# ThorsteinnJonsson/SLAM_framework

Hardware: AMD Instinct MI355X
Metric: stereo frames/sec ORB extract+match @1241x376, 2000 kp/frame (higher is better)
Workload: dtype u8; 1 GPU; configs[1]: synthetic 1241x376 stereo stream, 2000 kp/frame, extract L+R + stereo match + frame-to-frame match; batch=256, streams=1, batches_in_flight=2, nfeatures=2000, nlevels=8, parallelism=frame-sharded x1

## Files before the change

slam_framework_amd/csrc/match_kernels.hip:

```cpp
#include <hip/hip_runtime.h>
#include <stdint.h>

#include "device_math.h"
#include "timing.h"
#include "match_kernels.h"
#include "undistort.h"

namespace slamgpu {

#ifndef STEREO_LANES
#define STEREO_LANES 16
#endif

constexpr int TH_HIGH = 100, TH_LOW = 50, HISTO_LENGTH = 30;
constexpr uint64_t kNoKey = ~0ull;

__device__ __forceinline__ int hamming32(const uint8_t* a, const uint8_t* b) {
  const uint64_t* pa = reinterpret_cast<const uint64_t*>(a);
  const uint64_t* pb = reinterpret_cast<const uint64_t*>(b);
  return __popcll(pa[0] ^ pb[0]) + __popcll(pa[1] ^ pb[1]) + __popcll(pa[2] ^ pb[2]) +
         __popcll(pa[3] ^ pb[3]);
}

__device__ __forceinline__ const uint8_t* level_img(const ImageBatch& b, const OrbGeom* g,
                                                    int img, int level, int* pitch) {
  if (level == 0) {
    *pitch = b.in_pitch;
    return batch_image(b, img);
  }
  *pitch = g->lv[level].pitch;
  return b.pyr + (int64_t)img * g->pyr_bytes + g->lv[level].offset;
}

template <int CAP, int NT = 256>
__device__ int scan256(int* arr, int n, int* wsum) {
  constexpr int per = (CAP + NT - 1) / NT;
  const int lane = threadIdx.x & 63, wid = wave_id();
  const int base = threadIdx.x * per;
  int loc[per];
  int s = 0;
#pragma unroll
  for (int i = 0; i < per; i++) {
    loc[i] = (base + i < n) ? arr[base + i] : 0;
    s += loc[i];
  }
  int x = s;
#pragma unroll
  for (int off = 1; off < 64; off <<= 1) {
    const int y = __shfl_up(x, off, 64);
    if (lane >= off) x += y;
  }
  if (lane == 63) wsum[wid] = x;
  __syncthreads();
  int pre = 0, tot = 0;
#pragma unroll
  for (int w = 0; w < NT / 64; w++) {
    pre += (w < wid) ? wsum[w] : 0;
    tot += wsum[w];
  }
  pre += x - s;
#pragma unroll
  for (int i = 0; i < per; i++) {
    if (base + i < n) arr[base + i] = pre;
    pre += loc[i];
  }
  __syncthreads();
  return tot;
}

__device__ __forceinline__ uint32_t wave_or(uint32_t v) {
#pragma unroll
  for (int off = 32; off >= 1; off >>= 1) v |= __shfl_xor(v, off, 64);
  return v;
}

constexpr int kMaxRows = 2048;

template <int NT>
__device__ __forceinline__ void stereo_rows_body(int f, const OrbGeom* __restrict__ g,
                                                 const FrameKps& ext, int nrows,
                                                 const StereoWorkspace& ws,
                                                 uint32_t* __restrict__ err) {
  __shared__ int cnt[kMaxRows + 1];
  __shared__ int wsum[NT / 64];
  const int tid = threadIdx.x;
  const int ir = 2 * f + 1;
  const KeyPoint* kr = ext.kps + ir * ext.stride;
  const int nr = ext.n[ir * ext.n_stride];
  int* rs = ws.row_start + (int64_t)f * (nrows + 1);
  uint2* items = ws.row_items + (int64_t)f * ws.row_cap;
  for (int i = tid; i <= nrows; i += NT) cnt[i] = 0;
  __syncthreads();
  constexpr int kChunk = 2048 / NT;
  uint2 kit[kChunk];
  auto row_span = [&](int base, int (&lo)[kChunk], int (&hi)[kChunk]) {
    float ky[kChunk];
    int ko[kChunk];
#pragma unroll
    for (int u = 0; u < kChunk; u++) {
      const int i = base + NT * u + tid;
      ky[u] = 0.0f;
      ko[u] = -1;
      if (i < nr) {
        ky[u] = kr[i].y;
        ko[u] = kr[i].octave;
        kit[u] = make_uint2((uint32_t)i | (uint32_t)ko[u] << 16, __float_as_uint(kr[i].x));
      }
    }
#pragma unroll
    for (int u = 0; u < kChunk; u++) {
      lo[u] = 0;
      hi[u] = -1;
      if (ko[u] >= 0) {
        const float r = 2.0f * g->lv[ko[u]].scale;
        lo[u] = max((int)floorf(ky[u] - r), 0);
        hi[u] = min((int)ceilf(ky[u] + r), nrows - 1);
      }
    }
  };
  for (int base = 0; base < nr; base += NT * kChunk) {
    int lo[kChunk], hi[kChunk];
    row_span(base, lo, hi);
#pragma unroll
    for (int u = 0; u < kChunk; u++)
      for (int yi = lo[u]; yi <= hi[u]; ++yi) atomicAdd(&cnt[yi], 1);
  }
  __syncthreads();
  const int total = scan256<kMaxRows + 1, NT>(cnt, nrows, wsum);
  for (int i = tid; i < nrows; i += NT) rs[i] = cnt[i];
  if (tid == 0) {
    rs[nrows] = total;
    if (total > ws.row_cap) atomicOr(err, kErrRowOverflow);
  }
  __syncthreads();
  for (int base = 0; base < nr; base += NT * kChunk) {
    int lo[kChunk], hi[kChunk];
    row_span(base, lo, hi);
#pragma unroll
    for (int u = 0; u < kChunk; u++)
      for (int yi = lo[u]; yi <= hi[u]; ++yi) {
        const int pos = atomicAdd(&cnt[yi], 1);
        if (pos < ws.row_cap) items[pos] = kit[u];
      }
  }
}

template <int NT>
__global__ __launch_bounds__(NT) void stereo_rows_kernel(const OrbGeom* __restrict__ g,
                                                         FrameKps ext, int nrows,
                                                         StereoWorkspace ws,
                                                         uint32_t* __restrict__ err) {
  stereo_rows_body<NT>(blockIdx.x, g, ext, nrows, ws, err);
}

template <int G>
__device__ __forceinline__ uint32_t group_min(uint32_t v) {
#pragma unroll
  for (int off = G / 2; off >= 1; off >>= 1) {
    const uint32_t o = __shfl_xor(v, off, 64);
    v = o < v ? o : v;
  }
  return v;
}

template <int G>
__global__ __launch_bounds__(256) void stereo_match_kernel(ImageBatch b,
                                                           const OrbGeom* __restrict__ g,
                                                           FrameKps ext, Camera cam, int nrows,
                                                           StereoWorkspace ws, StereoOut out) {
  constexpr int NPW = 64 / G;
  constexpr int kRounds = (121 + G - 1) / G;
  int f, bx;
  xcd_image_block(&f, &bx);
  const int lane = threadIdx.x & 63, grp = lane / G, hl = lane % G;
  const int iL = (bx * 4 + wave_id()) * NPW + grp;
  const int il = 2 * f, ir = 2 * f + 1;
  const int nl = ext.n[il * ext.n_stride];
  const int64_t o = (int64_t)f * g->kp_cap + iL;
  bool ok = iL < nl;
  if (ok && hl == 0) {
    out.u_right[o] = -1.0f;
    out.depth[o] = -1.0f;
    ws.sad[o] = -1;
  }
  KeyPoint kpL{};
  if (ok) kpL = ext.kps[il * ext.stride + iL];
  const int levelL = kpL.octave;
  const float vL = kpL.y, uL = kpL.x;
  const int row = (int)vL;
  ok = ok && row >= 0 && row < nrows;
  const int* rs = ws.row_start + (int64_t)f * (nrows + 1);
  const uint2* items = ws.row_items + (int64_t)f * ws.row_cap;
  int c0 = 0, c1 = 0;
  if (ok) {
    c0 = rs[row];
    c1 = min(rs[row + 1], ws.row_cap);
  }
  ok = ok && c0 < c1;
  const float baseline = cam.bf / cam.fx;
  const float minZ = baseline, minD = 0, maxD = cam.bf / minZ;
  const float minU = uL - maxD, maxU = uL - minD;
  ok = ok && !(maxU < 0);
  const uint8_t* dL = ext.desc + (il * ext.stride + (ok ? iL : 0)) * 32;
  const uint8_t* dRb = ext.desc + ir * ext.stride * 32;
  uint32_t best = ((uint32_t)TH_HIGH << 16) | 0xffffu;
  float bestU = 0.0f;
  if (ok) {
    constexpr int kCandU = 2;
    const uint4* dLq = reinterpret_cast<const uint4*>(dL);
    const uint4 l0 = dLq[0], l1 = dLq[1];
    for (int cb = c0 + hl; cb < c1; cb += G * kCandU) {
      int iR[kCandU];
      float uR[kCandU];
      bool pass[kCandU];
#pragma unroll
      for (int u = 0; u < kCandU; u++) {
        const int c = cb + G * u;
        const uint2 it = c < c1 ? items[c] : make_uint2(0xffffffffu, 0u);
        iR[u] = (int)(it.x & 0xffffu);
        const int oct = (int)(it.x >> 16);
        uR[u] = __uint_as_float(it.y);
        pass[u] = c < c1 && oct >= levelL - 1 && oct <= levelL + 1 && uR[u] >= minU &&
                  uR[u] <= maxU;
      }
      uint4 r0[kCandU], r1[kCandU];
#pragma unroll
      for (int u = 0; u < kCandU; u++)
        if (pass[u]) {
          const uint4* dr = reinterpret_cast<const uint4*>(dRb + iR[u] * 32);
          r0[u] = dr[0];
          r1[u] = dr[1];
        }
#pragma unroll
      for (int u = 0; u < kCandU; u++)
        if (pass[u]) {
          const int dist = __popc(l0.x ^ r0[u].x) + __popc(l0.y ^ r0[u].y) + __popc(l0.z ^ r0[u].z) +
                           __popc(l0.w ^ r0[u].w) + __popc(l1.x ^ r1[u].x) + __popc(l1.y ^ r1[u].y) +
                           __popc(l1.z ^ r1[u].z) + __popc(l1.w ^ r1[u].w);
          const uint32_t key = ((uint32_t)dist << 16) | (uint32_t)iR[u];
          if (dist < TH_HIGH && key < best) {
            best = key;
            bestU = uR[u];
          }
        }
    }
  }
  const uint32_t mine = best;
  best = group_min<G>(best);
  const uint64_t gmask = (G == 64 ? ~0ull : ((1ull << G) - 1ull)) << (G * grp);
  const uint64_t hit = __ballot(mine == best) & gmask;
  const float uRbest = __shfl(bestU, hit ? __builtin_ctzll(hit) : lane, 64);
  const int bestDist = (int)(best >> 16);
  const int thOrbDist = (TH_HIGH + TH_LOW) / 2;
  ok = ok && bestDist < thOrbDist;
  const float uR0 = ok ? uRbest : 0.f;
  const float scaleFactor = g->lv[levelL].inv_scale;
  const float scaleduL = roundf(kpL.x * scaleFactor);
  const float scaledvL = roundf(kpL.y * scaleFactor);
  const float scaleduR0 = roundf(uR0 * scaleFactor);
  const int w = 5, L = 5;
  const LevelGeom& LG = g->lv[levelL];
  const float iniu = scaleduR0 + L - w;
  const float endu = scaleduR0 + L + w + 1;
  ok = ok && !(iniu < 0 || endu >= (float)LG.w);
  const int yc = (int)scaledvL, xcl = (int)scaleduL, xcr = (int)scaleduR0;
  ok = ok && !(yc - w < 0 || yc + w >= LG.h || xcl - w < 0 || xcl + w >= LG.w || xcr - L - w < 0);
  __shared__ int s_part[4][NPW][128];
  __shared__ uint32_t s_win[4][NPW][11][11];
  int* part = s_part[wave_id()][grp];
  uint32_t(*win)[11] = s_win[wave_id()][grp];
  int pl = 0, pr = 0;
  const uint8_t* IL = nullptr;
  const uint8_t* IR = nullptr;
  if (ok) {
    IL = level_img(b, g, il, levelL, &pl);
    IR = level_img(b, g, ir, levelL, &pr);
  }
  const int al = (xcl - w) & ~3, ar = (xcr - L - w) & ~3;
  const bool dw = ((((uintptr_t)IL | (uintptr_t)IR) | (uintptr_t)(pl | pr)) & 3) == 0;
  const int lastw = (LG.w - 1) >> 2;
  if (ok) {
#pragma unroll
    for (int rnd = 0; rnd < kRounds; rnd++) {
      const int p = hl + G * rnd;
      if (p < 121) {
        const int r = p / 11, d = p - 11 * r;
        const bool left = d < 4;
        const uint8_t* img = left ? IL : IR;
        const int pitch = left ? pl : pr;
        const int x0 = left ? al + 4 * d : ar + 4 * (d - 4);
        const uint8_t* rowp = img + (int64_t)(yc - w + r) * pitch;
        uint32_t v;
        if (dw) {
          v = reinterpret_cast<const uint32_t*>(rowp)[min(x0 >> 2, lastw)];
        } else {
          v = 0;
          for (int j = 0; j < 4; j++)
            v |= (uint32_t)rowp[min(x0 + j, LG.w - 1)] << (8 * j);
        }
        win[r][d] = v;
      }
    }
  }
  __builtin_amdgcn_fence(__ATOMIC_SEQ_CST, "wavefront");
  __builtin_amdgcn_wave_barrier();
  const uint8_t* wb = reinterpret_cast<const uint8_t*>(&win[0][0]);
  if (ok) {
    const uint32_t* ww = &win[0][0];
    const int oL = xcl - w - al, oR0 = xcr - L - w - ar;
    const int cl = wb[44 * w + (xcl - al)];
    constexpr uint32_t kBias = 0x02020202u;
#pragma unroll
    for (int rnd = 0; rnd < kRounds; rnd++) {
      const int p = hl + G * rnd;
      if (p < 121) {
        const int k = p / 11, yr = p - 11 * k;
        const int cr = wb[44 * w + 16 + (xcr + k - L - ar)];
        const uint32_t* rowL = ww + 11 * yr;
        const int oR = oR0 + k;
        const uint32_t* rowR = rowL + 4 + (oR >> 2);
        const uint32_t l0 = rowL[0], l1 = rowL[1], l2 = rowL[2], l3 = rowL[3];
        const uint32_t r0 = rowR[0], r1 = rowR[1], r2 = rowR[2], r3 = rowR[3];
        const uint32_t a[3] = {__builtin_amdgcn_alignbyte(l1, l0, oL),
                               __builtin_amdgcn_alignbyte(l2, l1, oL),
                               __builtin_amdgcn_alignbyte(l3, l2, oL)};
        const uint32_t bsh = (uint32_t)(oR & 3);
        const uint32_t bb[3] = {__builtin_amdgcn_alignbyte(r1, r0, bsh),
                                __builtin_amdgcn_alignbyte(r2, r1, bsh),
                                __builtin_amdgcn_alignbyte(r3, r2, bsh)};
        typedef unsigned short u16x2_t __attribute__((ext_vector_type(2)));
        const unsigned short d = (unsigned short)(cl - cr);
        const u16x2_t dd = {d, d}, dlast = {d, 0};
        uint32_t acc = 0;
#pragma unroll
        for (int j = 0; j < 6; j++) {
          const uint32_t sel = j == 5 ? 0x04040402u : (j & 1) ? 0x04030402u : 0x05010400u;
          const uint32_t A = __builtin_amdgcn_perm(kBias, a[j >> 1], sel);
          const u16x2_t B = __builtin_bit_cast(u16x2_t, __builtin_amdgcn_perm(kBias, bb[j >> 1], sel)) +
                            (j == 5 ? dlast : dd);
          acc = __builtin_amdgcn_sad_u16(A, __builtin_bit_cast(uint32_t, B), acc);
        }
        part[p] = (int)acc;
      }
    }
  }
  __builtin_amdgcn_fence(__ATOMIC_SEQ_CST, "wavefront");
  __builtin_amdgcn_wave_barrier();
  int sad = 0x7fffffff;
  if (ok && hl < 2 * L + 1) {
    int acc = 0;
#pragma unroll
    for (int yy = 0; yy < 2 * w + 1; yy++) acc += part[11 * hl + yy];
    sad = acc;
  }
  float vDists[11];
#pragma unroll
  for (int k = 0; k < 11; k++) vDists[k] = (float)__shfl(sad, G * grp + k, 64);
  if (!ok || hl != 0) return;
  int bestSad = 0x7fffffff, bestincR = 0;
#pragma unroll
  for (int k = 0; k < 11; k++) {
    if (vDists[k] < (float)bestSad) {
      bestSad = (int)vDists[k];
      bestincR = k - L;
    }
  }
  if (bestincR == -L || bestincR == L) return;
  const float dist1 = vDists[L + bestincR - 1];
  const float dist2 = vDists[L + bestincR];
  const float dist3 = vDists[L + bestincR + 1];
  const float deltaR = (dist1 - dist3) / (2.0f * (dist1 + dist3 - 2.0f * dist2));
  if (deltaR < -1 || deltaR > 1) return;
  float bestuR = LG.scale * ((float)scaleduR0 + (float)bestincR + deltaR);
  float disparity = (uL - bestuR);
  if (disparity >= minD && disparity < maxD) {
    if (disparity <= 0) {
      disparity = 0.01f;
      bestuR = uL - 0.01f;
    }
    out.depth[o] = cam.bf / disparity;
    out.u_right[o] = bestuR;
    ws.sad[o] = bestSad;
  }
}

template <int NT>
__global__ __launch_bounds__(NT) void stereo_median_kernel(const OrbGeom* __restrict__ g,
                                                           FrameKps ext, StereoWorkspace ws,
                                                           StereoOut out,
                                                           uint8_t* __restrict__ pack,
                                                           const uint32_t* __restrict__ err) {
  constexpr int kCap = 4096;
  __shared__ uint32_t vals[kCap];
  __shared__ int hist[256];
  __shared__ int n_valid, s_digit, s_rank;
  __shared__ uint32_t s_or;
  const int f = blockIdx.x, tid = threadIdx.x, lane = tid & 63;
  const int nl = min(ext.n[2 * f * ext.n_stride], kCap);
  const int64_t base = (int64_t)f * g->kp_cap;
  if (tid == 0) {
    n_valid = 0;
    s_or = 0;
  }
  __syncthreads();
  uint32_t vor = 0;
  for (int i0 = 0; i0 < nl; i0 += NT * 4) {
    int sv[4];
#pragma unroll
    for (int u = 0; u < 4; u++) {
      const int i = i0 + NT * u + tid;
      sv[u] = i < nl ? ws.sad[base + i] : -1;
    }
#pragma unroll
    for (int u = 0; u < 4; u++)
      if (sv[u] >= 0) {
        vals[atomicAdd(&n_valid, 1)] = (uint32_t)sv[u];
        vor |= (uint32_t)sv[u];
      }
  }
  vor = wave_or(vor);
  if (lane == 0 && vor) atomicOr(&s_or, vor);
  __syncthreads();
  const int n = n_valid;
  const uint32_t all_or = s_or;
  uint32_t prefix = 0, mask = 0;
  int k = n / 2;
  const int top = all_or >> 24 ? 24 : all_or >> 16 ? 16 : all_or >> 8 ? 8 : 0;
  for (int shift = top; shift >= 0 && n > 0; shift -= 8) {
    if (tid < 256) hist[tid] = 0;
    __syncthreads();
    for (int i = tid; i < n; i += NT) {
      const uint32_t v = vals[i];
      if ((v & mask) == prefix) atomicAdd(&hist[(v >> shift) & 255u], 1);
    }
    __syncthreads();
    if (tid < 64) {
      int h[4], sum = 0;
#pragma unroll
      for (int j = 0; j < 4; j++) {
        h[j] = hist[4 * lane + j];
        sum += h[j];
      }
      int x = sum;
#pragma unroll
      for (int off = 1; off < 64; off <<= 1) {
        const int y = __shfl_up(x, off, 64);
        if (lane >= off) x += y;
      }
      const int before = x - sum;
      if (before <= k && k < x) {
        int acc = before, d = 0;
#pragma unroll
        for (int j = 0; j < 4; j++)
          if (d == 0 && acc + h[j] > k) d = j + 1;
          else if (d == 0) acc += h[j];
        s_digit = 4 * lane + d - 1;
        s_rank = k - acc;
      }
    }
    __syncthreads();
    prefix |= (uint32_t)s_digit << shift;
    mask |= 255u << shift;
    k = s_rank;
    __syncthreads();
  }
  const float median = (float)(int)prefix;
  const float thDist = (1.5f * 1.4f) * median;
  const size_t kc = (size_t)g->kp_cap;
  float* const pur = pack && f == 0
                         ? reinterpret_cast<float*>(pack + 16 + 2 * kc * sizeof(KeyPoint) + 2 * kc * 32)
                         : nullptr;
  const int nall = pur ? min(max(ext.n[0], 0), (int)kc) : nl;
  for (int i = tid; i < nall; i += NT) {
    const int s = i < nl ? ws.sad[base + i] : -1;
    if (n > 0 && s >= 0 && !((float)s < thDist)) {
      out.u_right[base + i] = -1.0f;
      out.depth[base + i] = -1.0f;
      ws.sad[base + i] = -1;
      if (pur) pur[i] = pur[kc + i] = -1.0f;
    } else if (pur) {
      pur[i] = out.u_right[base + i];
      pur[kc + i] = out.depth[base + i];
    }
  }
  __syncthreads();
  if (pur && tid == 0) reinterpret_cast<uint32_t*>(pack)[2] = *err;
}

__device__ __forceinline__ void frame_pack_body(const FrameKps& ext,
                                                const float* __restrict__ u_right,
                                                const float* __restrict__ depth,
                                                const uint32_t* __restrict__ err, int kp_cap,
                                                uint8_t* __restrict__ dst, int parts, int gid,
                                                int gsz) {
  const int c0 = ext.n[0], c1 = ext.n[ext.n_stride];
  const int n0 = min(max(c0, 0), kp_cap), n1 = min(max(c1, 0), kp_cap);
  const size_t kc = (size_t)kp_cap;
  if (gid == 0) {
    int* h = reinterpret_cast<int*>(dst);
    if (parts & 1) {
      h[0] = c0;
      h[1] = c1;
      h[3] = (int)*err;
    }
    if (parts & 2) h[2] = (int)*err;
  }
  auto copy = [&](const void* src, size_t dst_off, int words) {
    const uint32_t* s = reinterpret_cast<const uint32_t*>(src);
    uint32_t* d = reinterpret_cast<uint32_t*>(dst + dst_off);
    for (int i = gid; i < words; i += gsz) d[i] = s[i];
  };
  const size_t kps_off = 16, desc_off = kps_off + 2 * kc * sizeof(KeyPoint);
  const size_t ur_off = desc_off + 2 * kc * 32, dp_off = ur_off + kc * sizeof(float);
  if (parts & 1) {
    copy(ext.kps, kps_off, 7 * n0);
    copy(ext.kps + ext.stride, kps_off + kc * sizeof(KeyPoint), 7 * n1);
    copy(ext.desc, desc_off, 8 * n0);
    copy(ext.desc + 32 * ext.stride, desc_off + 32 * kc, 8 * n1);
  }
  if (parts & 2) {
    copy(u_right, ur_off, n0);
    copy(depth, dp_off, n0);
  }
}
__global__ __launch_bounds__(256) void frame_pack_kernel(FrameKps ext,
                                                         const float* __restrict__ u_right,
                                                         const float* __restrict__ depth,
                                                         const uint32_t* __restrict__ err,
                                                         int kp_cap, uint8_t* __restrict__ dst,
                                                         int parts) {
  frame_pack_body(ext, u_right, depth, err, kp_cap, dst, parts,
                  blockIdx.x * blockDim.x + threadIdx.x, gridDim.x * blockDim.x);
}

void launch_frame_pack(const FrameKps& ext, const float* u_right, const float* depth,
                       const uint32_t* err, int kp_cap, uint8_t* dst, hipStream_t st, int parts) {
  static_assert(sizeof(KeyPoint) == 28, "keypoint layout");
  SLAMGPU_LAUNCH("frame_pack", st, frame_pack_kernel, dim3(32), dim3(256), 0, st, ext, u_right,
                 depth, err, kp_cap, dst, parts);
}

__global__ void trace_marker_kernel() {}

void launch_trace_marker(int id, hipStream_t st) {
  hipLaunchKernelGGL(trace_marker_kernel, dim3(1, id), dim3(64), 0, st);
}

void launch_stereo(const ImageBatch& b, const OrbGeomDev& gd, const Camera& cam, int n_frames,
                   const StereoWorkspace& ws, const StereoOut& out, hipStream_t st,
                   uint8_t* pack, bool rows_done) {
  const OrbGeom& g = *gd.host;
  FrameKps ext{gd.out.kps, gd.out.desc, gd.out.nkps, g.kp_cap, 1};
  const int nrows = g.lv[0].h;
  if (rows_done) {
  } else if (n_frames <= 8)
    SLAMGPU_LAUNCH("stereo_rows", st, stereo_rows_kernel<1024>, dim3(n_frames), dim3(1024), 0, st,
                   gd.dev, ext, nrows, ws, gd.ws.err);
  else
    SLAMGPU_LAUNCH("stereo_rows", st, stereo_rows_kernel<256>, dim3(n_frames), dim3(256), 0, st,
                   gd.dev, ext, nrows, ws, gd.ws.err);
  constexpr int kG = STEREO_LANES, kPerBlock = 4 * (64 / kG);
  SLAMGPU_LAUNCH("stereo_match", st, stereo_match_kernel<kG>,
                 dim3((g.kp_cap + kPerBlock - 1) / kPerBlock, n_frames), dim3(256), 0, st, b,
                 gd.dev, ext, cam, nrows, ws, out);
  if (n_frames <= 8)
    SLAMGPU_LAUNCH("stereo_median", st, stereo_median_kernel<1024>, dim3(n_frames), dim3(1024), 0,
                   st, gd.dev, ext, ws, out, pack, gd.ws.err);
  else
    SLAMGPU_LAUNCH("stereo_median", st, stereo_median_kernel<256>, dim3(n_frames), dim3(256), 0,
                   st, gd.dev, ext, ws, out, pack, gd.ws.err);
}

__device__ __forceinline__ int grid_cell(const Camera& cam, float x, float y) {
  const int px = (int)roundf((x - cam.min_x) / cam.cell_w);
  const int py = (int)roundf((y - cam.min_y) / cam.cell_h);
  if (px < 0 || px >= kGridCols || py < 0 || py >= kGridRows) return -1;
  return px * kGridRows + py;
}

template <int NT>
__device__ __forceinline__ void grid_build_body(int f, const FrameKps& cur, const Camera& cam,
                                                int kp_cap, const GridWorkspace& gw) {
  __shared__ int cnt[kGridCells + 1];
  __shared__ int wsum[NT / 64];
  const int tid = threadIdx.x;
  const KeyPoint* k = cur.kps + f * cur.stride;
  const int n = cur.n[f * cur.n_stride];
  int* cs = gw.cell_start + (int64_t)f * (kGridCells + 1);
  uint4* items = gw.cell_items + (int64_t)f * kp_cap;
  for (int i = tid; i <= kGridCells; i += NT) cnt[i] = 0;
  constexpr int kChunk = 2048 / NT;
  float kx[kChunk], ky[kChunk];
  int ko[kChunk];
  auto cells = [&](int base, int (&c)[kChunk]) {
#pragma unroll
    for (int u = 0; u < kChunk; u++) {
      const int i = base + NT * u + tid;
      kx[u] = ky[u] = 0.0f;
      ko[u] = 0;
      if (i < n) {
        kx[u] = k[i].x;
        ky[u] = k[i].y;
        ko[u] = k[i].octave;
      }
    }
#pragma unroll
    for (int u = 0; u < kChunk; u++)
      c[u] = base + NT * u + tid < n ? grid_cell(cam, kx[u], ky[u]) : -1;
  };
  __syncthreads();
  for (int base = 0; base < n; base += NT * kChunk) {
    int c[kChunk];
    cells(base, c);
#pragma unroll
    for (int u = 0; u < kChunk; u++)
      if (c[u] >= 0) atomicAdd(&cnt[c[u]], 1);
  }
  __syncthreads();
  const int total = scan256<kGridCells + 1, NT>(cnt, kGridCells, wsum);
  for (int i = tid; i < kGridCells; i += NT) cs[i] = cnt[i];
  if (tid == 0) cs[kGridCells] = total;
  __syncthreads();
  for (int base = 0; base < n; base += NT * kChunk) {
    int c[kChunk];
    cells(base, c);
#pragma unroll
    for (int u = 0; u < kChunk; u++)
      if (c[u] >= 0)
        items[atomicAdd(&cnt[c[u]], 1)] =
            make_uint4((uint32_t)(base + NT * u + tid) | (uint32_t)ko[u] << 16,
                       __float_as_uint(kx[u]), __float_as_uint(ky[u]), 0u);
  }
}
__global__ __launch_bounds__(256) void grid_build_kernel(FrameKps cur, Camera cam, int kp_cap,
                                                         GridWorkspace gw) {
  grid_build_body<256>(blockIdx.x, cur, cam, kp_cap, gw);
}

void launch_grid(const FrameKps& cur, const Camera& cam, int n_frames, int kp_cap,
                 const GridWorkspace& gw, hipStream_t st) {
  SLAMGPU_LAUNCH("grid_build", st, grid_build_kernel, dim3(n_frames), dim3(256), 0, st, cur, cam,
                 kp_cap, gw);
}

__global__ __launch_bounds__(1024) void frame_aux_kernel(const OrbGeom* __restrict__ g,
                                                         FrameKps ext, int nrows,
                                                         StereoWorkspace ws, uint32_t* err,
                                                         FrameKps left, Camera cam, int kp_cap,
                                                         GridWorkspace gw, uint8_t* pack) {
  switch (blockIdx.y) {
    case 0: stereo_rows_body<1024>(0, g, ext, nrows, ws, err); break;
    case 1: grid_build_body<1024>(0, left, cam, kp_cap, gw); break;
    default:
      frame_pack_body(ext, nullptr, nullptr, err, kp_cap, pack, 1, threadIdx.x, 1024);
      break;
  }
}

void launch_frame_aux(const OrbGeomDev& gd, const FrameKps& left, const Camera& cam,
                      const GridWorkspace& gw, const StereoWorkspace& ws, uint8_t* pack,
                      hipStream_t st) {
  const OrbGeom& g = *gd.host;
  FrameKps ext{gd.out.kps, gd.out.desc, gd.out.nkps, g.kp_cap, 1};
  SLAMGPU_LAUNCH("frame_aux", st, frame_aux_kernel, dim3(1, 3), dim3(1024), 0, st, gd.dev, ext,
                 g.lv[0].h, ws, gd.ws.err, left, cam, g.kp_cap, gw, pack);
}

__global__ __launch_bounds__(256) void undistort_kernel(FrameKps src, KeyPoint* __restrict__ dst,
                                                        int64_t dst_stride, float fx, float fy,
                                                        float cx, float cy, Distortion dc) {
  const int f = blockIdx.y, i = blockIdx.x * 256 + threadIdx.x;
  if (i >= src.n[f * src.n_stride]) return;
  KeyPoint kp = src.kps[f * src.stride + i];
  if (dc.k[0] != 0.0f) undistort_point(fx, fy, cx, cy, dc, kp.x, kp.y, &kp.x, &kp.y);
  dst[f * dst_stride + i] = kp;
}

void launch_undistort(const FrameKps& src, KeyPoint* dst, int64_t dst_stride, const Camera& cam,
                      const Distortion& dc, int n_sets, int kp_cap, hipStream_t st) {
  SLAMGPU_LAUNCH("undistort", st, undistort_kernel, dim3((kp_cap + 255) / 256, n_sets), dim3(256),
                 0, st, src, dst, dst_stride, cam.fx, cam.fy, cam.cx, cam.cy, dc);
}

struct ScanCtx {
  float x, y, r;
  int min_level, max_level;
  float ur, gate;
  int max_dist;
  const uint8_t* desc;
};

struct FrameView {
  const KeyPoint* kps;
  const uint8_t* desc;
  const float* u_right;
  const int* cell_start;
  const uint4* cell_items;
  const uint8_t* blocked;
};

__device__ __forceinline__ uint32_t wave_min_key(uint32_t v) {
#pragma unroll
  for (int M = 32; M >= 1; M >>= 1) v = min(v, lane_partner_u32(v, M));
  return v;
}
__device__ __forceinline__ uint64_t wave_min_key(uint64_t v) {
#pragma unroll
  for (int M = 32; M >= 1; M >>= 1) {
    const uint64_t o = (uint64_t)lane_partner_u32((uint32_t)(v >> 32), M) << 32 |
                       lane_partner_u32((uint32_t)v, M);
    v = o < v ? o : v;
  }
  return v;
}
__device__ __forceinline__ int wave_sum_bfly(int v) {
#pragma unroll
  for (int M = 32; M >= 1; M >>= 1) v += (int)lane_partner_u32((uint32_t)v, M);
  return v;
}
__device__ __forceinline__ int wave_incl_scan(int v) {
  v += __builtin_amdgcn_update_dpp(0, v, 0x111, 0xf, 0xf, true);
  v += __builtin_amdgcn_update_dpp(0, v, 0x112, 0xf, 0xf, true);
  v += __builtin_amdgcn_update_dpp(0, v, 0x114, 0xf, 0xf, true);
  v += __builtin_amdgcn_update_dpp(0, v, 0x118, 0xf, 0xf, true);
  v += __builtin_amdgcn_update_dpp(0, v, 0x142, 0xa, 0xf, false);
  v += __builtin_amdgcn_update_dpp(0, v, 0x143, 0xc, 0xf, false);
  return v;
}

template <int G>
__device__ __forceinline__ int group_incl_scan(int v) {
  static_assert(G == 16 || G == 64, "groups are DPP rows or the wave");
  if constexpr (G == 64) {
    return wave_incl_scan(v);
  } else {
    v += __builtin_amdgcn_update_dpp(0, v, 0x111, 0xf, 0xf, true);
    v += __builtin_amdgcn_update_dpp(0, v, 0x112, 0xf, 0xf, true);
    v += __builtin_amdgcn_update_dpp(0, v, 0x114, 0xf, 0xf, true);
    v += __builtin_amdgcn_update_dpp(0, v, 0x118, 0xf, 0xf, true);
    return v;
  }
}
template <int G>
__device__ __forceinline__ uint32_t group_min_key(uint32_t v) {
#pragma unroll
  for (int M = G / 2; M >= 1; M >>= 1) v = min(v, lane_partner_u32(v, M));
  return v;
}
template <int G>
__device__ __forceinline__ uint64_t group_min_key(uint64_t v) {
#pragma unroll
  for (int M = G / 2; M >= 1; M >>= 1) {
    const uint64_t o = (uint64_t)lane_partner_u32((uint32_t)(v >> 32), M) << 32 |
                       lane_partner_u32((uint32_t)v, M);
    v = o < v ? o : v;
  }
  return v;
}
template <int G>
__device__ __forceinline__ int group_sum(int v) {
#pragma unroll
  for (int M = G / 2; M >= 1; M >>= 1) v += (int)lane_partner_u32((uint32_t)v, M);
  return v;
}

template <typename K>
__device__ __forceinline__ K scan_key(int dist, int cell, int i) {
  if constexpr (sizeof(K) == 4)
    return (uint32_t)dist << 23 | (uint32_t)cell << 11 | (uint32_t)i;
  else
    return ((uint64_t)dist << 32) | ((uint64_t)cell << 12) | (uint64_t)i;
}
template <typename K>
__device__ __forceinline__ uint64_t key64(K k) {
  if constexpr (sizeof(K) == 4)
    return k == ~0u ? kNoKey
                    : ((uint64_t)(k >> 23) << 32) | ((uint64_t)((k >> 11) & 0xfffu) << 12) |
                          (uint64_t)(k & 0x7ffu);
  else
    return k;
}

__device__ __forceinline__ int cell_floor(float v) { return (int)floorf(fminf(fmaxf(v, -1e6f), 1e6f)); }
__device__ __forceinline__ int cell_ceil(float v) { return (int)ceilf(fminf(fmaxf(v, -1e6f), 1e6f)); }

template <typename K, int G = 64>
__device__ int scan_query_k(const ScanCtx& c, const Camera& cam, const FrameView& F,
                            const uint32_t* claimed, uint64_t* top, int lane, bool skip = false) {
  const int gl = lane & (G - 1), gb = lane & ~(G - 1);
  int nMinCellX = 0, nMaxCellX = -1, nMinCellY = 0, nMaxCellY = -1;
  if (!skip) {
    nMinCellX = max(0, cell_floor((c.x - cam.min_x - c.r) / cam.cell_w));
    nMaxCellX = min(kGridCols - 1, cell_ceil((c.x - cam.min_x + c.r) / cam.cell_w));
    nMinCellY = max(0, cell_floor((c.y - cam.min_y - c.r) / cam.cell_h));
    nMaxCellY = min(kGridRows - 1, cell_ceil((c.y - cam.min_y + c.r) / cam.cell_h));
  }
  constexpr K kNone = (K)~(K)0;
  K t[kTopK];
#pragma unroll
  for (int k = 0; k < kTopK; k++) t[k] = kNone;
  int cnt = 0;
  if (!(nMaxCellX < 0 || nMinCellX >= kGridCols || nMaxCellY < 0 || nMinCellY >= kGridRows)) {
    const bool bCheckLevels = (c.min_level > 0) || (c.max_level >= 0);
    const int ny = nMaxCellY - nMinCellY + 1;
    const int total = (nMaxCellX - nMinCellX + 1) * ny;
    for (int cb = 0; cb < total; cb += G) {
      const int ci = cb + gl;
      int cell = 0, q0 = 0, nq = 0;
      if (ci < total) {
        const int ix = nMinCellX + ci / ny, iy = nMinCellY + ci % ny;
        cell = ix * kGridRows + iy;
        q0 = F.cell_start[cell];
        nq = F.cell_start[cell + 1] - q0;
      }
      const int incl = group_incl_scan<G>(nq);
      const int excl = incl - nq;
      const int npairs = G == 64 ? __builtin_amdgcn_readlane(incl, 63) : __shfl(incl, gb + G - 1, 64);
      for (int k0 = 0; k0 < npairs; k0 += G) {
        const int k = k0 + gl;
        int lo = 0;
#pragma unroll
        for (int step = G / 2; step >= 1; step >>= 1) {
          const int cand = lo + step;
          const int ec = __shfl(excl, gb + (cand & (G - 1)), 64);
          if (cand < G && ec <= k) lo = cand;
        }
        const int p = __shfl(q0, gb + lo, 64) + (k - __shfl(excl, gb + lo, 64));
        const int pcell = __shfl(cell, gb + lo, 64);
        if (k >= npairs) continue;
        const uint4 it = F.cell_items[p];
        const int i = (int)(it.x & 0xffffu), octave = (int)(it.x >> 16);
        if (bCheckLevels) {
          if (octave < c.min_level) continue;
          if (c.max_level >= 0 && octave > c.max_level) continue;
        }
        const float distx = __uint_as_float(it.y) - c.x, disty = __uint_as_float(it.z) - c.y;
        if (!(fabsf(distx) < c.r && fabsf(disty) < c.r)) continue;
        const bool blk = F.blocked[i] != 0;
        const float ur = F.u_right[i];
        const int dist = hamming32(c.desc, F.desc + i * 32);
        if (blk) continue;
        if (claimed && (claimed[i >> 5] >> (i & 31)) & 1u) continue;
        if (ur > 0 && fabsf(c.ur - ur) > c.gate) continue;
        if (dist > c.max_dist) continue;
        const K key = scan_key<K>(dist, pcell, i);
        cnt++;
        if (key < t[kTopK - 1]) {
          t[kTopK - 1] = key;
#pragma unroll
          for (int k2 = kTopK - 1; k2 > 0; k2--)
            if (t[k2] < t[k2 - 1]) {
              const K s2 = t[k2];
              t[k2] = t[k2 - 1];
              t[k2 - 1] = s2;
            }
        }
      }
    }
  }
#pragma unroll
  for (int k = 0; k < kTopK; k++) top[k] = kNoKey;
#pragma unroll
  for (int k = 0; k < kTopK; k++) {
    const K m = G == 64 ? wave_min_key(t[0]) : group_min_key<G>(t[0]);
// ... 486 lines not shown
```

Measured before the change: 112,000 stereo frames/s.

## Compute stereo SAD per window row in registers with buffer loads and DPP reduction

Rewrites the SAD refinement stage of the stereo match kernel. Each lane of a 16-lane group now loads one window row directly into registers with raw buffer loads and computes all 11 shift SADs for that row. Partial sums are reduced across lanes with DPP row shifts instead of staging windows and partials in LDS. It also adds an early exit for blocks past the keypoint count and consolidates the output writes. The kernel is now hard-wired to 16 lanes, and it relies on buffer bounds checks to make the previous clamping of out-of-range reads unnecessary.

```diff
diff --git a/slam_framework_amd/csrc/match_kernels.hip b/slam_framework_amd/csrc/match_kernels.hip
--- a/slam_framework_amd/csrc/match_kernels.hip
+++ b/slam_framework_amd/csrc/match_kernels.hip
@@ -7,10 +7,6 @@
 #include "undistort.h"
 
 namespace slamgpu {
-
-#ifndef STEREO_LANES
-#define STEREO_LANES 16
-#endif
 
 constexpr int TH_HIGH = 100, TH_LOW = 50, HISTO_LENGTH = 30;
 constexpr uint64_t kNoKey = ~0ull;
@@ -20,16 +16,6 @@
   const uint64_t* pb = reinterpret_cast<const uint64_t*>(b);
   return __popcll(pa[0] ^ pb[0]) + __popcll(pa[1] ^ pb[1]) + __popcll(pa[2] ^ pb[2]) +
          __popcll(pa[3] ^ pb[3]);
-}
-
-__device__ __forceinline__ const uint8_t* level_img(const ImageBatch& b, const OrbGeom* g,
-                                                    int img, int level, int* pitch) {
-  if (level == 0) {
-    *pitch = b.in_pitch;
-    return batch_image(b, img);
-  }
-  *pitch = g->lv[level].pitch;
-  return b.pyr + (int64_t)img * g->pyr_bytes + g->lv[level].offset;
 }
 
 template <int CAP, int NT = 256>
@@ -163,26 +149,35 @@
   return v;
 }
 
+typedef uint32_t u32x4_t __attribute__((ext_vector_type(4)));
+typedef uint32_t u32x3_t __attribute__((ext_vector_type(3)));
+
+__device__ __forceinline__ uint32_t byte_pair(const uint32_t* e, int p) {
+  const int q = p >> 2;
+  switch (p & 3) {
+    case 0: return __builtin_amdgcn_perm(0u, e[q], 0x0c010c00u);
+    case 1: return __builtin_amdgcn_perm(0u, e[q], 0x0c020c01u);
+    case 2: return __builtin_amdgcn_perm(0u, e[q], 0x0c030c02u);
+    default: return __builtin_amdgcn_perm(e[q + 1], e[q], 0x0c040c03u);
+  }
+}
+
 template <int G>
 __global__ __launch_bounds__(256) void stereo_match_kernel(ImageBatch b,
                                                            const OrbGeom* __restrict__ g,
                                                            FrameKps ext, Camera cam, int nrows,
                                                            StereoWorkspace ws, StereoOut out) {
+  static_assert(G == 16, "the SAD stage puts a keypoint's 11 window rows on one 16-lane DPP row");
   constexpr int NPW = 64 / G;
-  constexpr int kRounds = (121 + G - 1) / G;
   int f, bx;
   xcd_image_block(&f, &bx);
+  const int il = 2 * f, ir = 2 * f + 1;
+  const int nl = ext.n[il * ext.n_stride];
+  if (bx * 4 * NPW >= nl) return;
   const int lane = threadIdx.x & 63, grp = lane / G, hl = lane % G;
   const int iL = (bx * 4 + wave_id()) * NPW + grp;
-  const int il = 2 * f, ir = 2 * f + 1;
-  const int nl = ext.n[il * ext.n_stride];
-  const int64_t o = (int64_t)f * g->kp_cap + iL;
-  bool ok = iL < nl;
-  if (ok && hl == 0) {
-    out.u_right[o] = -1.0f;
-    out.depth[o] = -1.0f;
-    ws.sad[o] = -1;
-  }
+  const bool valid = iL < nl;
+  bool ok = valid;
   KeyPoint kpL{};
   if (ok) kpL = ext.kps[il * ext.stride + iL];
   const int levelL = kpL.octave;
@@ -265,98 +260,103 @@
   ok = ok && !(iniu < 0 || endu >= (float)LG.w);
   const int yc = (int)scaledvL, xcl = (int)scaleduL, xcr = (int)scaleduR0;
   ok = ok && !(yc - w < 0 || yc + w >= LG.h || xcl - w < 0 || xcl + w >= LG.w || xcr - L - w < 0);
-  __shared__ int s_part[4][NPW][128];
-  __shared__ uint32_t s_win[4][NPW][11][11];
-  int* part = s_part[wave_id()][grp];
-  uint32_t(*win)[11] = s_win[wave_id()][grp];
-  int pl = 0, pr = 0;
-  const uint8_t* IL = nullptr;
-  const uint8_t* IR = nullptr;
-  if (ok) {
-    IL = level_img(b, g, il, levelL, &pl);
-    IR = level_img(b, g, ir, levelL, &pr);
-  }
-  const int al = (xcl - w) & ~3, ar = (xcr - L - w) & ~3;
-  const bool dw = ((((uintptr_t)IL | (uintptr_t)IR) | (uintptr_t)(pl | pr)) & 3) == 0;
-  const int lastw = (LG.w - 1) >> 2;
-  if (ok) {
-#pragma unroll
-    for (int rnd = 0; rnd < kRounds; rnd++) {
-      const int p = hl + G * rnd;
-      if (p < 121) {
-        const int r = p / 11, d = p - 11 * r;
-        const bool left = d < 4;
-        const uint8_t* img = left ? IL : IR;
-        const int pitch = left ? pl : pr;
-        const int x0 = left ? al + 4 * d : ar + 4 * (d - 4);
-        const uint8_t* rowp = img + (int64_t)(yc - w + r) * pitch;
-        uint32_t v;
-        if (dw) {
-          v = reinterpret_cast<const uint32_t*>(rowp)[min(x0 >> 2, lastw)];
-        } else {
-          v = 0;
-          for (int j = 0; j < 4; j++)
-            v |= (uint32_t)rowp[min(x0 + j, LG.w - 1)] << (8 * j);
-        }
-        win[r][d] = v;
-      }
-    }
-  }
-  __builtin_amdgcn_fence(__ATOMIC_SEQ_CST, "wavefront");
-  __builtin_amdgcn_wave_barrier();
-  const uint8_t* wb = reinterpret_cast<const uint8_t*>(&win[0][0]);
-  if (ok) {
-    const uint32_t* ww = &win[0][0];
-    const int oL = xcl - w - al, oR0 = xcr - L - w - ar;
-    const int cl = wb[44 * w + (xcl - al)];
-    constexpr uint32_t kBias = 0x02020202u;
-#pragma unroll
-    for (int rnd = 0; rnd < kRounds; rnd++) {
-      const int p = hl + G * rnd;
-      if (p < 121) {
-        const int k = p / 11, yr = p - 11 * k;
-        const int cr = wb[44 * w + 16 + (xcr + k - L - ar)];
-        const uint32_t* rowL = ww + 11 * yr;
-        const int oR = oR0 + k;
-        const uint32_t* rowR = rowL + 4 + (oR >> 2);
-        const uint32_t l0 = rowL[0], l1 = rowL[1], l2 = rowL[2], l3 = rowL[3];
-        const uint32_t r0 = rowR[0], r1 = rowR[1], r2 = rowR[2], r3 = rowR[3];
-        const uint32_t a[3] = {__builtin_amdgcn_alignbyte(l1, l0, oL),
-                               __builtin_amdgcn_alignbyte(l2, l1, oL),
-                               __builtin_amdgcn_alignbyte(l3, l2, oL)};
-        const uint32_t bsh = (uint32_t)(oR & 3);
-        const uint32_t bb[3] = {__builtin_amdgcn_alignbyte(r1, r0, bsh),
-                                __builtin_amdgcn_alignbyte(r2, r1, bsh),
-                                __builtin_amdgcn_alignbyte(r3, r2, bsh)};
-        typedef unsigned short u16x2_t __attribute__((ext_vector_type(2)));
-        const unsigned short d = (unsigned short)(cl - cr);
-        const u16x2_t dd = {d, d}, dlast = {d, 0};
-        uint32_t acc = 0;
-#pragma unroll
-        for (int j = 0; j < 6; j++) {
-          const uint32_t sel = j == 5 ? 0x04040402u : (j & 1) ? 0x04030402u : 0x05010400u;
-          const uint32_t A = __builtin_amdgcn_perm(kBias, a[j >> 1], sel);
-          const u16x2_t B = __builtin_bit_cast(u16x2_t, __builtin_amdgcn_perm(kBias, bb[j >> 1], sel)) +
-                            (j == 5 ? dlast : dd);
-          acc = __builtin_amdgcn_sad_u16(A, __builtin_bit_cast(uint32_t, B), acc);
-        }
-        part[p] = (int)acc;
-      }
-    }
-  }
-  __builtin_amdgcn_fence(__ATOMIC_SEQ_CST, "wavefront");
-  __builtin_amdgcn_wave_barrier();
-  int sad = 0x7fffffff;
-  if (ok && hl < 2 * L + 1) {
-    int acc = 0;
-#pragma unroll
-    for (int yy = 0; yy < 2 * w + 1; yy++) acc += part[11 * hl + yy];
-    sad = acc;
-  }
+  const int64_t o = (int64_t)f * g->kp_cap + iL;
+  if (valid && !ok && hl == 0) {
+    out.u_right[o] = -1.0f;
+    out.depth[o] = -1.0f;
+    ws.sad[o] = -1;
+  }
+  if (!ok) return;
+  const LevelGeom& L0 = g->lv[0];
+  const uint8_t* const img_l = batch_image(b, il);
+  const uint8_t* const img_r = batch_image(b, ir);
+  const bool dw = ((((uintptr_t)img_l | (uintptr_t)img_r) | (uintptr_t)b.in_pitch) & 3) == 0;
+  const int bytes0 = __builtin_amdgcn_readfirstlane((L0.h - 1) * b.in_pitch +
+                                                    (dw ? (L0.w + 3) & ~3 : L0.w));
+  const int bytesp = __builtin_amdgcn_readfirstlane((int)g->pyr_bytes);
+  const __amdgpu_buffer_rsrc_t rs_l0 = buf_rsrc(img_l, bytes0), rs_r0 = buf_rsrc(img_r, bytes0);
+  const __amdgpu_buffer_rsrc_t rs_lp = buf_rsrc(b.pyr + (int64_t)il * g->pyr_bytes, bytesp);
+  const __amdgpu_buffer_rsrc_t rs_rp = buf_rsrc(b.pyr + (int64_t)ir * g->pyr_bytes, bytesp);
+  const int al = (xcl - 5) & ~3, ar = (xcr - 10) & ~3;
+  const int wy = yc - 5 + min(hl, 10);
+  uint32_t lw[4], rw[7];
+  auto rows = [&](__amdgpu_buffer_rsrc_t rl, __amdgpu_buffer_rsrc_t rr, int ol, int orr) {
+    const u32x4_t l4 = __builtin_amdgcn_raw_buffer_load_b128(rl, ol, 0, 0);
+    const u32x4_t r4 = __builtin_amdgcn_raw_buffer_load_b128(rr, orr, 0, 0);
+    const u32x3_t r3 = __builtin_amdgcn_raw_buffer_load_b96(rr, orr + 16, 0, 0);
+#pragma unroll
+    for (int i = 0; i < 4; i++) lw[i] = l4[i], rw[i] = r4[i];
+#pragma unroll
+    for (int i = 0; i < 3; i++) rw[4 + i] = r3[i];
+  };
+  if (levelL != 0) {
+    const int ro = (int)LG.offset + wy * LG.pitch;
+    rows(rs_lp, rs_rp, ro + al, ro + ar);
+  } else if (dw) {
+    const int ro = wy * b.in_pitch;
+    rows(rs_l0, rs_r0, ro + al, ro + ar);
+  } else {
+    const int ro = wy * b.in_pitch;
+#pragma unroll
+    for (int i = 0; i < 4; i++) {
+      lw[i] = 0;
+#pragma unroll
+      for (int j = 0; j < 4; j++)
+        lw[i] |= (uint32_t)__builtin_amdgcn_raw_buffer_load_b8(rs_l0, ro + al + 4 * i + j, 0, 0)
+                 << (8 * j);
+    }
+#pragma unroll
+    for (int i = 0; i < 7; i++) {
+      rw[i] = 0;
+#pragma unroll
+      for (int j = 0; j < 4; j++)
+        rw[i] |= (uint32_t)__builtin_amdgcn_raw_buffer_load_b8(rs_r0, ro + ar + 4 * i + j, 0, 0)
+                 << (8 * j);
+    }
+  }
+  const uint32_t oL = (uint32_t)(xcl - 5 - al), oR = (uint32_t)(xcr - 10 - ar);
+  uint32_t a[3], e[6], ec[6];
+#pragma unroll
+  for (int i = 0; i < 3; i++) a[i] = __builtin_amdgcn_alignbyte(lw[i + 1], lw[i], oL);
+#pragma unroll
+  for (int i = 0; i < 6; i++) e[i] = __builtin_amdgcn_alignbyte(rw[i + 1], rw[i], oR);
+  const uint32_t ac = __shfl(a[1], 5, G);
+#pragma unroll
+  for (int i = 0; i < 6; i++) ec[i] = i >= 1 && i <= 3 ? __shfl(e[i], 5, G) : 0u;
+  constexpr uint32_t kBias = 0x02020202u;
+  constexpr uint32_t kBias2 = 0x02000200u;
+  uint32_t A[6];
+#pragma unroll
+  for (int j = 0; j < 5; j++)
+    A[j] = __builtin_amdgcn_perm(kBias, a[j >> 1], (j & 1) ? 0x04030402u : 0x05010400u);
+  A[5] = __builtin_amdgcn_perm(ac, a[2], 0x0c050c02u) + kBias2;
+  const uint32_t C = __builtin_amdgcn_perm(0u, ac, 0x0c010c01u) + kBias2;
+  int S[11];
+#pragma unroll
+  for (int k = 0; k < 11; k++) {
+    const int c = k + 5, hc = c & 3, p = k + 10, h = p & 3;
+    const uint32_t crr =
+        __builtin_amdgcn_perm(0u, ec[c >> 2], 0x0c000c00u | (uint32_t)hc | (uint32_t)hc << 16);
+    const uint32_t dd = C - crr;
+    uint32_t acc = 0;
+#pragma unroll
+    for (int j = 0; j < 5; j++)
+      acc = __builtin_amdgcn_sad_u16(A[j], byte_pair(e, k + 2 * j) + dd, acc);
+    const uint32_t last = __builtin_amdgcn_perm(
+        ec[c >> 2], e[p >> 2], 0x0c000c00u | (uint32_t)h | (uint32_t)(4 + hc) << 16);
+    S[k] = (int)__builtin_amdgcn_sad_u16(A[5], last + dd, acc);
+  }
+#pragma unroll
+  for (int k = 0; k < 11; k++) {
+    S[k] += __builtin_amdgcn_update_dpp(0, S[k], 0x111, 0xf, 0xf, true);
+    S[k] += __builtin_amdgcn_update_dpp(0, S[k], 0x112, 0xf, 0xf, true);
+    S[k] += __builtin_amdgcn_update_dpp(0, S[k], 0x114, 0xf, 0xf, true);
+    S[k] += __builtin_amdgcn_update_dpp(0, S[k], 0x118, 0xf, 0xf, true);
+  }
+  if (hl != 10) return;
   float vDists[11];
 #pragma unroll
-  for (int k = 0; k < 11; k++) vDists[k] = (float)__shfl(sad, G * grp + k, 64);
-  if (!ok || hl != 0) return;
+  for (int k = 0; k < 11; k++) vDists[k] = (float)S[k];
   int bestSad = 0x7fffffff, bestincR = 0;
 #pragma unroll
   for (int k = 0; k < 11; k++) {
@@ -365,23 +365,30 @@
       bestincR = k - L;
     }
   }
-  if (bestincR == -L || bestincR == L) return;
-  const float dist1 = vDists[L + bestincR - 1];
-  const float dist2 = vDists[L + bestincR];
-  const float dist3 = vDists[L + bestincR + 1];
-  const float deltaR = (dist1 - dist3) / (2.0f * (dist1 + dist3 - 2.0f * dist2));
-  if (deltaR < -1 || deltaR > 1) return;
-  float bestuR = LG.scale * ((float)scaleduR0 + (float)bestincR + deltaR);
-  float disparity = (uL - bestuR);
-  if (disparity >= minD && disparity < maxD) {
-    if (disparity <= 0) {
-      disparity = 0.01f;
-      bestuR = uL - 0.01f;
-    }
-    out.depth[o] = cam.bf / disparity;
-    out.u_right[o] = bestuR;
-    ws.sad[o] = bestSad;
-  }
+  float o_ur = -1.0f, o_depth = -1.0f;
+  int o_sad = -1;
+  if (!(bestincR == -L || bestincR == L)) {
+    const float dist1 = vDists[L + bestincR - 1];
+    const float dist2 = vDists[L + bestincR];
+    const float dist3 = vDists[L + bestincR + 1];
+    const float deltaR = (dist1 - dist3) / (2.0f * (dist1 + dist3 - 2.0f * dist2));
+    if (!(deltaR < -1 || deltaR > 1)) {
+      float bestuR = LG.scale * ((float)xcr + (float)bestincR + deltaR);
+      float disparity = (uL - bestuR);
+      if (disparity >= minD && disparity < maxD) {
+        if (disparity <= 0) {
+          disparity = 0.01f;
+          bestuR = uL - 0.01f;
+        }
+        o_depth = cam.bf / disparity;
+        o_ur = bestuR;
+        o_sad = bestSad;
+      }
+    }
+  }
+  out.u_right[o] = o_ur;
+  out.depth[o] = o_depth;
+  ws.sad[o] = o_sad;
 }
 
 template <int NT>
@@ -559,7 +566,7 @@
   else
     SLAMGPU_LAUNCH("stereo_rows", st, stereo_rows_kernel<256>, dim3(n_frames), dim3(256), 0, st,
                    gd.dev, ext, nrows, ws, gd.ws.err);
-  constexpr int kG = STEREO_LANES, kPerBlock = 4 * (64 / kG);
+  constexpr int kG = 16, kPerBlock = 4 * (64 / kG);
   SLAMGPU_LAUNCH("stereo_match", st, stereo_match_kernel<kG>,
                  dim3((g.kp_cap + kPerBlock - 1) / kPerBlock, n_frames), dim3(256), 0, st, b,
                  gd.dev, ext, cam, nrows, ws, out);
```

New measurement: 119,200 stereo frames/s (median of 6 runs). +6.4%, better.
